# yigolden/JpegLibrary

Measured on AMD Instinct MI355X. Metric: Mpixels/s decoded, 4K 4:2:0 baseline Q75 RST=4, 1 & 8 GPU vs CPU ref, higher is better.
Workload: dtype f32; 1 GPU; 1024 x 3840x2160 420 baseline Q75 DRI=4 per GPU, output interleaved_u8 resident in HBM; images_per_gpu=1024

## Files before the change

jpeglibrary_amd/csrc/k3_idct.hip:

```cpp
#include <hip/hip_runtime.h>
#include <stdint.h>

#include <algorithm>
#include <atomic>
#include <cstdio>
#include <cstdlib>

#include "common.h"
#include "kernels.h"
#include "encode_kernels.h"
#include "kernels_device.h"

namespace jpgpu {


__device__ constexpr uint8_t kNat[64] = {0,  1,  8,  16, 9,  2,  3,  10, 17, 24, 32, 25, 18, 11, 4,  5,  12, 19, 26, 33, 40, 48,
                                         41, 34, 27, 20, 13, 6,  7,  14, 21, 28, 35, 42, 49, 56, 57, 50, 43, 36, 29, 22, 15, 23,
                                         30, 37, 44, 51, 58, 59, 52, 45, 38, 31, 39, 46, 53, 60, 61, 54, 47, 55, 62, 63};

static_assert(kIdctBlocksPerWg == 256, "the split form's reciprocals are exact for tiles of up to 256 blocks");
static_assert(kMaxBlocksPerMcu == 16, "kRecip16 and the 16-bit reciprocals of the split form cover 1..16 blocks per MCU");
__device__ constexpr uint32_t kRecip16[kMaxBlocksPerMcu + 1] = {0, 65536, 32768, 21846, 16384, 13108, 10923, 9363, 8192, 7282, 6554, 5958, 5462, 5042, 4682, 4370, 4096};

#define JPGPU_IDCT8(y0, y1, y2, y3, y4, y5, y6, y7)                     \
    {                                                                   \
        float mz0 = y1 + y7;                                            \
        float mz2 = y3 + y7;                                            \
        float mz1 = y3 + y5;                                            \
        float mz3 = y1 + y5;                                            \
        float mz4 = (mz0 + mz1) * 1.175875602f;                         \
        mz2 = (mz2 * -1.961570560f) + mz4;                              \
        mz3 = (mz3 * -0.390180644f) + mz4;                              \
        mz0 = mz0 * -0.899976223f;                                      \
        mz1 = mz1 * -2.562915447f;                                      \
        const float mb3 = ((y7 * 0.298631336f) + mz0) + mz2;            \
        const float mb2 = ((y5 * 2.053119869f) + mz1) + mz3;            \
        const float mb1 = ((y3 * 3.072711026f) + mz1) + mz2;            \
        const float mb0 = ((y1 * 1.501321110f) + mz0) + mz3;            \
        mz4 = (y2 + y6) * 0.541196100f;                                 \
        mz0 = y0 + y4;                                                  \
        mz1 = y0 - y4;                                                  \
        mz2 = mz4 + (y6 * -1.847759065f);                               \
        mz3 = mz4 + (y2 * 0.765366865f);                                \
        const float a0 = mz0 + mz3;                                     \
        const float a3 = mz0 - mz3;                                     \
        const float a1 = mz1 + mz2;                                     \
        const float a2 = mz1 - mz2;                                     \
        y0 = a0 + mb0;                                                  \
        y7 = a0 - mb0;                                                  \
        y1 = a1 + mb1;                                                  \
        y6 = a1 - mb1;                                                  \
        y2 = a2 + mb2;                                                  \
        y5 = a2 - mb2;                                                  \
        y3 = a3 + mb3;                                                  \
        y4 = a3 - mb3;                                                  \
    }

__device__ __forceinline__ void block_dequant(const uint8_t *c_lds, uint32_t swz, const uint16_t *q_lds, float (&f)[64]) {
#pragma unroll
    for (int piece = 0; piece < 8; piece++) {
        const uint4 cv = *reinterpret_cast<const uint4 *>(c_lds + ((piece ^ swz) * 16));
        const uint4 qv = reinterpret_cast<const uint4 *>(q_lds)[piece];
        const uint32_t cw[4] = {cv.x, cv.y, cv.z, cv.w};
        const uint32_t qw[4] = {qv.x, qv.y, qv.z, qv.w};
#pragma unroll
        for (int j = 0; j < 8; j++) {
            const int k = piece * 8 + j;
            const uint32_t w = cw[j >> 1], q = qw[j >> 1];
            const int32_t c = (j & 1) ? ((int32_t)w >> 16) : (int32_t)(int16_t)(w & 0xFFFF);
            const int32_t qq = (j & 1) ? (int32_t)(q >> 16) : (int32_t)(q & 0xFFFF);
            f[kNat[k]] = (float)(qq * c);
        }
    }
}

typedef float float2v __attribute__((ext_vector_type(2)));
typedef short short2v __attribute__((ext_vector_type(2)));
typedef unsigned short ushort2v __attribute__((ext_vector_type(2)));

template <typename T>
__device__ __forceinline__ void idct8(T &y0, T &y1, T &y2, T &y3, T &y4, T &y5, T &y6, T &y7) {
    T mz0 = y1 + y7;
    T mz2 = y3 + y7;
    T mz1 = y3 + y5;
    T mz3 = y1 + y5;
    T mz4 = (mz0 + mz1) * 1.175875602f;
    mz2 = (mz2 * -1.961570560f) + mz4;
    mz3 = (mz3 * -0.390180644f) + mz4;
    mz0 = mz0 * -0.899976223f;
    mz1 = mz1 * -2.562915447f;
    const T mb3 = ((y7 * 0.298631336f) + mz0) + mz2;
    const T mb2 = ((y5 * 2.053119869f) + mz1) + mz3;
    const T mb1 = ((y3 * 3.072711026f) + mz1) + mz2;
    const T mb0 = ((y1 * 1.501321110f) + mz0) + mz3;
// ... 127 lines not shown
            *reinterpret_cast<uint4 *>(dst + i * 4) = v;
        }
    } else {
        uint32_t w[N * 3 / 4];
#pragma unroll
        for (int i = 0; i < N; i += 4) {
            w[i * 3 / 4 + 0] = p[i] | (p[i + 1] << 24);
            w[i * 3 / 4 + 1] = (p[i + 1] >> 8) | (p[i + 2] << 16);
            w[i * 3 / 4 + 2] = (p[i + 2] >> 16) | (p[i + 3] << 8);
        }
        if (N == 16) {
#pragma unroll
            for (int i = 0; i < 3; i++) {
                const uint4 v = {w[i * 4], w[i * 4 + 1], w[i * 4 + 2], w[i * 4 + 3]};
                *reinterpret_cast<uint4 *>(dst + i * 16) = v;
            }
        } else {
#pragma unroll
            for (int i = 0; i < N * 3 / 8; i++) {
                const uint2 v = {w[i * 2], w[i * 2 + 1]};
                *reinterpret_cast<uint2 *>(dst + i * 8) = v;
            }
        }
    }
}

__global__ __launch_bounds__(256) void ycc_to_rgb_kernel(const uint8_t *__restrict__ src, uint8_t *__restrict__ dst, uint64_t n_pixels, int comps,
                                                         int bpp, YccRgbFactors k) {
    for (uint64_t i = (uint64_t)blockIdx.x * 256 + threadIdx.x; i < n_pixels; i += (uint64_t)gridDim.x * 256) {
        const uint32_t y = src[i * comps];
        const uint32_t cb = comps == 3 ? src[i * 3 + 1] : 128u, cr = comps == 3 ? src[i * 3 + 2] : 128u;
        const uint32_t px = rgb_pixel(y, chroma_terms(cb, cr, k));
        uint8_t *d = dst + i * bpp;
        d[0] = (uint8_t)px;
        d[1] = (uint8_t)(px >> 8);
        d[2] = (uint8_t)(px >> 16);
        if (bpp == 4) d[3] = 255;
    }
}

__global__ __launch_bounds__(256) void extend_u16_kernel(const uint8_t *__restrict__ planes, uint8_t *__restrict__ out_base,
                                                         const ExtendPlanes *__restrict__ images) {
    const ExtendPlanes g = images[blockIdx.y];
    uint16_t *out = reinterpret_cast<uint16_t *>(out_base + g.out_off);
    for (uint64_t px = (uint64_t)blockIdx.x * 256 + threadIdx.x; px < (uint64_t)g.width * g.height; px += (uint64_t)gridDim.x * 256) {
    const uint32_t y = (uint32_t)(px / g.width), x = (uint32_t)(px - (uint64_t)y * g.width);
    const uint32_t p = g.precision < 1u ? 1u : (g.precision > 16u ? 16u : g.precision), mx = (1u << p) - 1u;
    uint16_t v4[4] = {0, 0, 0, 0};
#pragma unroll
    for (uint32_t c = 0; c < 4u; c++) {
        if (c >= g.ncomp) continue;
        const int16_t *pl = reinterpret_cast<const int16_t *>(planes + g.plane_off[c]);
        const uint32_t mw = 8u * (g.max_h | (g.max_h == 0)), mh = 8u * (g.max_v | (g.max_v == 0));
        const uint32_t mcx = x / mw, pxm = x - mcx * mw, mcy = y / mh, pym = y - mcy * mh;
        const uint32_t bx = (pxm >> 3) < g.hcnt[c] - 1u ? (pxm >> 3) : g.hcnt[c] - 1u, by = (pym >> 3) < g.vcnt[c] - 1u ? (pym >> 3) : g.vcnt[c] - 1u;
        const uint32_t dx = pxm - 8u * bx, dy = pym - 8u * by;
        if (g.max_h != 0 && (dx >= (8u << g.hshift[c]) || dy >= (8u << g.vshift[c]))) continue;
        const uint32_t s = g.max_h == 0 ? (uint32_t)(uint16_t)pl[(uint64_t)(y >> g.vshift[c]) * g.pitch[c] + (x >> g.hshift[c])]
                                        : (uint32_t)(uint16_t)pl[(uint64_t)((mcy * g.vcnt[c] + by) * 8u + (dy >> g.vshift[c])) * g.pitch[c] + (mcx * g.hcnt[c] + bx) * 8u + (dx >> g.hshift[c])];
        uint32_t bits = s < mx ? s : mx;
        if (p >= 8u) {
            const uint32_t rem = 16u - p;
            bits = (bits << rem) | (bits & ((1u << rem) - 1u));
        } else {
            uint32_t cur = p;
            while (cur < 16u) {
                bits = (bits << p) | bits;
                cur += p;
            }
            if (cur > 16u) {
                bits >>= p;
                cur -= p;
                const uint32_t rem = 16u - cur;
                bits = (bits << rem) | (bits & ((1u << rem) - 1u));
            }
        }
        v4[c] = (uint16_t)bits;
    }
    *reinterpret_cast<uint2 *>(out + px * 4) = uint2{(uint32_t)v4[0] | ((uint32_t)v4[1] << 16), (uint32_t)v4[2] | ((uint32_t)v4[3] << 16)};
    }
}

template <int LAY, int CONV>
__device__ __forceinline__ void interleaved_output_from_tile(const uint8_t *sh_px, const DevScan &s, uint32_t tile_first, uint32_t n_mcu,
                                                             uint32_t tid, bool have_block, const DevScanComponent &comp, uint32_t mcu_x,
                                                             uint32_t mcu_y, uint32_t b, uint8_t *out, const YccRgbFactors &kf, bool reached,
                                                             uint32_t mcu, uint32_t fail_block) {
    const uint32_t W = s.width, H = s.height, C = s.frame_components;
    uint8_t *img = out + s.out_off;

    if (LAY == kLayGeneric) {
        if (have_block) {
            const uint32_t hs = comp.hs, vs = comp.vs;
            const bool flush = s.kind == kScanFrameOnly;
            const uint32_t x0 = flush ? (mcu_x * comp.h + s.blk_x[b]) * hs * 8 : (mcu_x * s.max_h + s.blk_x[b]) * 8;
            const uint32_t y0 = flush ? (mcu_y * comp.v + s.blk_y[b]) * vs * 8 : (mcu_y * s.max_v + s.blk_y[b]) * 8;
            const uint32_t hshift = 31 - __builtin_clz(hs | 1), vshift = 31 - __builtin_clz(vs | 1);
            const uint32_t bx = s.blk_x[b], by = s.blk_y[b];
            const bool overlap_h = !flush && comp.h > 1 && hs > 1, overlap_v = !flush && comp.v > 1 && vs > 1;
            const uint32_t base = b - (by * comp.h + bx);
            if ((overlap_h || overlap_v) && !reached) return;
            for (uint32_t v = 0; v < vs; v++)
                for (uint32_t i = 0; i < 8; i++) {
                    const uint32_t y = y0 + 8 * v + i;
                    if (y >= H) continue;
                    const uint8_t *srow = sh_px + ((8 * v + i) >> vshift) * kPxRowStride + tid * 8;
                    for (uint32_t h = 0; h < hs; h++) {
                        if (overlap_h || overlap_v) {
                            uint32_t later = 0xFFFFFFFFu;
                            if (overlap_h && bx + 1 < comp.h && h >= 1) later = base + by * comp.h + bx + 1;
                            else if (overlap_v && by + 1 < comp.v && v >= 1) {
                                const int32_t xf = (int32_t)bx + (int32_t)h - (int32_t)hs + 1;
                                later = base + (by + 1) * comp.h + (uint32_t)(xf < 0 ? 0 : xf);
                            }
                            if (later != 0xFFFFFFFFu && (uint64_t)mcu * s.blocks_per_mcu + later < fail_block) continue;
                        }
                        for (uint32_t j = 0; j < 8; j++) {
                            const uint32_t x = x0 + 8 * h + j;
                            if (x < W) img[((size_t)y * W + x) * C + comp.component_index] = srow[(8 * h + j) >> hshift];
                        }
                    }
                }
        }
    } else {
    constexpr uint32_t max_h = (LAY == kLayYccH1V1) ? 1 : 2;
    constexpr uint32_t max_v = (LAY == kLayYccH2V2) ? 2 : 1;
    constexpr uint32_t rows_per_mcu = 8 * max_v;
    constexpr uint32_t vshift = max_v >> 1;
    constexpr uint32_t kbpm = max_h * max_v + 2;
    const uint32_t n_tasks = rows_per_mcu * n_mcu;
    for (uint32_t t = tid; t < n_tasks; t += kIdctThreads) {
        const uint32_t row = t / n_mcu, m = t - row * n_mcu;
        const uint32_t gm = tile_first + m;
        const uint32_t gx = gm % s.mcus_per_line, gy = gm / s.mcus_per_line;
        const uint32_t y = gy * rows_per_mcu + row;
        if (y >= H) continue;
        const uint8_t *yrow = sh_px + (row & 7) * kPxRowStride + (m * kbpm + (row >> 3) * max_h) * 8;
        const uint8_t *crow = sh_px + (row >> vshift) * kPxRowStride + (m * kbpm + max_h * max_v) * 8;
        if (max_h == 2 && CONV != 0) {
            const uint4 yv = *reinterpret_cast<const uint4 *>(yrow);
            const uint4 cv = *reinterpret_cast<const uint4 *>(crow);
            uint32_t px[16];
#pragma unroll
            for (int j = 0; j < 8; j++) {
                const ChromaTerms t = chroma_terms(byte_of(cv.x, cv.y, j), byte_of(cv.z, cv.w, j), kf);
                px[2 * j] = rgb_pixel(byte_of(j < 4 ? yv.x : yv.z, j < 4 ? yv.y : yv.w, (2 * j) & 7), t);
                px[2 * j + 1] = rgb_pixel(byte_of(j < 4 ? yv.x : yv.z, j < 4 ? yv.y : yv.w, (2 * j + 1) & 7), t);
            }
            store_rgb_pixels<16, (CONV == 4 ? 4 : 3)>(img + ((size_t)y * W + gx * 16) * (CONV == 4 ? 4 : 3), px);
        } else if (CONV != 0) {
            const uint2 yv = *reinterpret_cast<const uint2 *>(yrow);
            const uint2 bv = *reinterpret_cast<const uint2 *>(crow);
            const uint2 rv = *reinterpret_cast<const uint2 *>(crow + 8);
            uint32_t px[8];
#pragma unroll
            for (int j = 0; j < 8; j++) px[j] = rgb_pixel(byte_of(yv.x, yv.y, j), chroma_terms(byte_of(bv.x, bv.y, j), byte_of(rv.x, rv.y, j), kf));
            store_rgb_pixels<8, (CONV == 4 ? 4 : 3)>(img + ((size_t)y * W + gx * 8) * (CONV == 4 ? 4 : 3), px);
        } else if (max_h == 2) {
            const uint4 yv = *reinterpret_cast<const uint4 *>(yrow);
            const uint4 cv = *reinterpret_cast<const uint4 *>(crow);
            const uint32_t cc0 = pick4(cv.x, cv.z, JPGPU_SEL(0, 4, 1, 5)), cc1 = pick4(cv.x, cv.z, JPGPU_SEL(2, 6, 3, 7));
            const uint32_t cc2 = pick4(cv.y, cv.w, JPGPU_SEL(0, 4, 1, 5)), cc3 = pick4(cv.y, cv.w, JPGPU_SEL(2, 6, 3, 7));
            uint4 o0, o1, o2;
            o0.x = pick4(yv.x, cc0, JPGPU_SEL(0, 4, 5, 1));
            o0.y = pick4(yv.x, cc0, JPGPU_SEL(4, 5, 2, 6));
            o0.z = pick4(yv.x, cc0, JPGPU_SEL(7, 3, 6, 7));
            o0.w = pick4(yv.y, cc1, JPGPU_SEL(0, 4, 5, 1));
            o1.x = pick4(yv.y, cc1, JPGPU_SEL(4, 5, 2, 6));
            o1.y = pick4(yv.y, cc1, JPGPU_SEL(7, 3, 6, 7));
            o1.z = pick4(yv.z, cc2, JPGPU_SEL(0, 4, 5, 1));
            o1.w = pick4(yv.z, cc2, JPGPU_SEL(4, 5, 2, 6));
            o2.x = pick4(yv.z, cc2, JPGPU_SEL(7, 3, 6, 7));
            o2.y = pick4(yv.w, cc3, JPGPU_SEL(0, 4, 5, 1));
            o2.z = pick4(yv.w, cc3, JPGPU_SEL(4, 5, 2, 6));
            o2.w = pick4(yv.w, cc3, JPGPU_SEL(7, 3, 6, 7));
            uint4 *dst = reinterpret_cast<uint4 *>(img + ((size_t)y * W + gx * 16) * 3);
            dst[0] = o0;
            dst[1] = o1;
            dst[2] = o2;
        } else {
            const uint2 yv = *reinterpret_cast<const uint2 *>(yrow);
            const uint2 bv = *reinterpret_cast<const uint2 *>(crow);
            const uint2 rv = *reinterpret_cast<const uint2 *>(crow + 8);
            uint2 o0, o1, o2;
            {
                const uint32_t lo = pick4(bv.x, rv.x, JPGPU_SEL(0, 4, 1, 5)), hi = pick4(bv.x, rv.x, JPGPU_SEL(2, 6, 3, 7));
                const uint32_t mid = pick4(lo, hi, JPGPU_SEL(2, 3, 4, 5));
                o0.x = pick4(yv.x, lo, JPGPU_SEL(0, 4, 5, 1));
                o0.y = pick4(yv.x, mid, JPGPU_SEL(4, 5, 2, 6));
                o1.x = pick4(yv.x, hi, JPGPU_SEL(5, 3, 6, 7));
            }
            {
                const uint32_t lo = pick4(bv.y, rv.y, JPGPU_SEL(0, 4, 1, 5)), hi = pick4(bv.y, rv.y, JPGPU_SEL(2, 6, 3, 7));
                const uint32_t mid = pick4(lo, hi, JPGPU_SEL(2, 3, 4, 5));
                o1.y = pick4(yv.y, lo, JPGPU_SEL(0, 4, 5, 1));
                o2.x = pick4(yv.y, mid, JPGPU_SEL(4, 5, 2, 6));
                o2.y = pick4(yv.y, hi, JPGPU_SEL(5, 3, 6, 7));
            }
            uint2 *dst = reinterpret_cast<uint2 *>(img + ((size_t)y * W + gx * 8) * 3);
            dst[0] = o0;
            dst[1] = o1;
            dst[2] = o2;
        }
    }
    }
}

typedef __attribute__((address_space(3))) void jpgpu_lds_void;
typedef const __attribute__((address_space(1))) void jpgpu_gbl_void;

template <int FMT, int LAY, bool PRE, bool SPLIT = false>
__device__ __forceinline__ void idct_output_body(
    const int16_t *__restrict__ coefs, const DevScan *__restrict__ scans, const IdctWork *__restrict__ work,
    const DevScanStatus *__restrict__ status, const DevQuantTable *__restrict__ quant_pool, uint8_t *__restrict__ out, YccRgbFactors kf) {
    constexpr int CONV = FMT == kFmtRgbU8 ? 3 : (FMT == kFmtRgbaU8 ? 4 : 0);
    constexpr bool kSampleBytes = fmt_is_sample_bytes(FMT);
    __shared__ __attribute__((aligned(16))) uint8_t sh_all[kIdctThreads * 128 + kIdctThreads * 64 + kMaxScanComponents * 128];
    uint8_t *sh = sh_all;
    uint8_t *sh_px = sh_all + kIdctThreads * 128;
    uint16_t(*sh_q)[64] = reinterpret_cast<uint16_t(*)[64]>(sh_all + kIdctThreads * 128 + kIdctThreads * 64);

    const IdctWork wk = work[blockIdx.x];
    const DevScan &s = scans[wk.scan];
    const uint32_t tid = threadIdx.x;
    const uint32_t wave = tid >> 6;
    const uint32_t bpm = s.blocks_per_mcu;
    const uint32_t mcus_per_tile = wk.mcus_per_tile;
    uint32_t decoded = status ? status[wk.scan].decoded_mcus : s.total_mcus;
    if (decoded > s.total_mcus) decoded = s.total_mcus;
    uint32_t fail_block = 0xFFFFFFFFu;
    if (status != nullptr && s.kind == kScanSequential) {
        const uint32_t fb = status[wk.scan].pad[1];
        if (fb != 0) fail_block = kFailBlockBase - fb;
        for (uint32_t j = s.first_scan; j < wk.scan; j++)
            if (scans[j].image_index == s.image_index && status[j].first_error != kNoError) fail_block = 0;
    }
    const bool keep = (s.shadow_mask & kKeepUnreachedMcus) != 0;
    constexpr bool kPerMcuLayout = fmt_is_interleaved(FMT) && (LAY == kLayYccH1V1 || LAY == kLayYccH2V1 || LAY == kLayYccH2V2);
    uint32_t first_mcu = wk.first_mcu;
    uint32_t range_end = wk.first_mcu + wk.n_mcus;
    if (first_mcu == kIdctPartialMcu) {
        if (fail_block == 0xFFFFFFFFu || fail_block % bpm == 0 || fail_block / bpm >= decoded) return;
        first_mcu = fail_block / bpm;
        range_end = first_mcu + 1;
    } else if (keep) {
        const uint32_t reach = kPerMcuLayout ? fail_block / bpm : (fail_block == 0xFFFFFFFFu ? fail_block : (fail_block + bpm - 1) / bpm);
        if (range_end > decoded) range_end = decoded;
        if (range_end > reach) range_end = reach;
        if (first_mcu >= range_end) return;
    }

    if (tid < (uint32_t)s.scan_components * 32) {
        const uint32_t c = tid >> 5, i = tid & 31;
        reinterpret_cast<uint32_t *>(sh_q[c])[i] =
            reinterpret_cast<const uint32_t *>(quant_pool[s.quant_pool[s.comp[c].quant_slot]].q)[i];
    }

    const uint32_t mcu_local = tid / bpm;
    const uint32_t b = tid - mcu_local * bpm;
    const uint32_t ci_early = s.blk_comp[b < kMaxBlocksPerMcu ? b : 0];
    const uint8_t *coef_bytes = reinterpret_cast<const uint8_t *>(coefs + s.coef_off * 64);

    auto tile_mcus = [&](uint32_t first) { return (range_end - first) < mcus_per_tile ? (range_end - first) : mcus_per_tile; };
    const uint32_t tile_blocks = mcus_per_tile * bpm;
    constexpr bool split = SPLIT && !PRE;
    if (split && (s.reserved0 & kScanSplitHandoff) == 0) return;
    const uint32_t sp_dri = split ? s.dri : 1u;
    const uint32_t sp_rb = kRecip16[bpm <= (uint32_t)kMaxBlocksPerMcu ? bpm : 0];
    const uint32_t sp_rd = __builtin_amdgcn_readfirstlane(sp_dri <= 256u ? ((1u << 20) + sp_dri - 1) / sp_dri : 0u);
    const uint32_t sp_w = sp_dri * bpm;
    const bool sp_fast = split && mcus_per_tile % (2 * sp_dri) == 0 && first_mcu % (2 * sp_dri) == 0;
    const uint32_t sp_rw = __builtin_amdgcn_readfirstlane((65536u + sp_w - 1) / sp_w);
    const uint8_t *sp_hi = coef_bytes + split_plane_lines(s.n_intervals, sp_dri, bpm) * 128;
    const uint8_t *sp_flags = reinterpret_cast<const uint8_t *>(reinterpret_cast<const uint64_t *>(coefs) + (s.reserved0 >> kSplitFlagShift));
    auto sp_locate = [&](uint32_t tile_first, uint32_t t, int k, uint32_t &line, uint32_t &iv, uint32_t &word) {
        const uint32_t i0 = __builtin_amdgcn_readfirstlane(tile_first / sp_dri), m0 = tile_first - i0 * sp_dri;
        const uint32_t blk = (uint32_t)k * 32 + (t >> 3);
        uint32_t q = (blk * sp_rb) >> 16;
        const uint32_t bb = blk - q * bpm;
        const uint32_t last = s.total_mcus - 1 - tile_first;
        q = q < last ? q : last;
        const uint32_t mm = m0 + q;
        const uint32_t by_mul = (mm * sp_rd) >> 20, by_cmp = mm >= sp_dri ? 1u : 0u;
        const uint32_t qi = sp_dri > 256u ? by_cmp : by_mul;
        const uint32_t m = mm - qi * sp_dri;
        iv = i0 + qi;
        line = ((iv >> 1) * sp_dri + m) * bpm + bb;
        word = ((iv >> 6) * sp_dri + m) * bpm + bb;
    };
    auto sp_locate_fast = [&](uint32_t i0, uint32_t t, int k, uint32_t &iv, uint32_t &word) {
        const uint32_t ll = (uint32_t)k * 16 + ((t >> 3) & 15u);
        const uint32_t pp = (ll * sp_rw) >> 16;
        iv = i0 + 2 * pp + ((t >> 7) & 1u);
        iv = iv < s.n_intervals ? iv : s.n_intervals - 1;
        word = (iv >> 6) * sp_w + (ll - pp * sp_w);
    };
    auto sp_own_block = [&](uint32_t t) {
        const uint32_t ml = (t * sp_rb) >> 16, bb = t - ml * bpm;
        const uint32_t ir = (ml * sp_rd) >> 20, m = ml - ir * sp_dri;
        const uint32_t ll = ((ir >> 1) * sp_dri + m) * bpm + bb;
        return ((ll >> 4) << 5) | ((ir & 1u) << 4) | (ll & 15u);
    };
    const uint32_t sp_ipt = __builtin_amdgcn_readfirstlane(mcus_per_tile / sp_dri);
    uint32_t sp_i0 = __builtin_amdgcn_readfirstlane(first_mcu / sp_dri);
    auto sp_load_flags = [&](uint32_t tile_first, uint32_t tile_i0, uint32_t (&fb)[8], uint32_t &bit_at) {
        uint32_t t_ = tid;
        asm volatile("" : "+v"(t_));
        bit_at = 0;
#pragma unroll
        for (int k = 0; k < 8; k++) {
            uint32_t line, iv, word;
            if (sp_fast) sp_locate_fast(tile_i0, t_, k, iv, word);
            else sp_locate(tile_first, t_, k, line, iv, word);
            fb[k] = sp_flags[word * 8 + ((iv >> 3) & 7u)];
            bit_at |= (iv & 7u) << (3 * k);
        }
    };
    auto sp_pack_flags = [&](uint32_t (&fb)[8], uint32_t bit_at) {
        uint32_t bits = 0;
#pragma unroll
        for (int k = 0; k < 8; k++) {
            asm volatile("" : "+v"(fb[k]));
            bits |= ((fb[k] >> ((bit_at >> (3 * k)) & 7u)) & 1u) << k;
        }
        return bits;
    };
    auto dma_tile = [&](uint32_t tile_first, uint32_t tile_i0, uint32_t hi_bits) {
        uint32_t t_ = tid;
        asm volatile("" : "+v"(t_));
        if (split && sp_fast) {
            const uint32_t piece = (t_ & 7) ^ ((t_ >> 4) & 7);
            const uint32_t slot = ((t_ >> 3) & 15u) * 2 + (t_ >> 7);
            const uint8_t *src = (piece < 4 ? coef_bytes : sp_hi) + (uint64_t)(tile_i0 >> 1) * sp_w * 128 + (slot * 64 + (piece & 3u) * 16);
            const uint8_t *zeros = sp_flags - 128 + (piece & 3u) * 16;
            const uint32_t fetch_bits = piece < 4 ? 0xFFu : hi_bits;
#pragma unroll
            for (int k = 0; k < 8; k++) {
                const uint8_t *from = ((fetch_bits >> k) & 1u) ? src + (uint32_t)(k * 2048) : zeros;
                if (k < 6 || (uint32_t)k * 32 + slot < tile_blocks)
                    __builtin_amdgcn_global_load_lds((jpgpu_gbl_void *)from, (jpgpu_lds_void *)(sh + ((uint32_t)k * kIdctThreads + wave * 64) * 16), 16, 0, 0);
            }
            return;
        }
        if (split) {
            const uint32_t piece = (t_ & 7) ^ ((t_ >> 4) & 7);
#pragma unroll
            for (int k = 0; k < 8; k++) {
                uint32_t line, iv, word;
                sp_locate(tile_first, t_, k, line, iv, word);
                const bool wanted = k < 6 || (uint32_t)k * 32 + (t_ >> 3) < tile_blocks;
                const bool fetch = wanted && (piece < 4 || ((hi_bits >> k) & 1u) != 0);
                const uint8_t *src = (piece < 4 ? coef_bytes : sp_hi) + ((uint64_t)line * 128 + (iv & 1u) * 64 + (piece & 3u) * 16);
                if (fetch)
                    __builtin_amdgcn_global_load_lds((jpgpu_gbl_void *)src, (jpgpu_lds_void *)(sh + ((uint32_t)k * kIdctThreads + wave * 64) * 16), 16, 0, 0);
                if (wanted && !fetch) *reinterpret_cast<uint4 *>(sh + ((uint32_t)k * kIdctThreads + t_) * 16) = uint4{0, 0, 0, 0};
            }
            return;
        }
        const uint32_t dma_lane_off = (t_ >> 3) * 128 + (((t_ & 7) ^ ((t_ >> 4) & 7)) * 16);
        const uint8_t *src = coef_bytes + (uint64_t)tile_first * bpm * 128;
#pragma unroll
        for (int k = 0; k < 8; k++)
            if (k < 6 || (uint32_t)k * 32 + (tid >> 3) < tile_blocks)
                __builtin_amdgcn_global_load_lds((jpgpu_gbl_void *)(src + (uint32_t)(k * 4096) + dma_lane_off),
                                                 (jpgpu_lds_void *)(sh + ((uint32_t)k * kIdctThreads + wave * 64) * 16), 16, 0, 0);
    };

    uint32_t hi_next = 0;
    if (split) {
        uint32_t fb[8], at;
        sp_load_flags(first_mcu, sp_i0, fb, at);
        asm volatile("s_waitcnt vmcnt(0)" ::: "memory");
        hi_next = sp_pack_flags(fb, at);
    }
    dma_tile(first_mcu, sp_i0, hi_next);
    if (split && first_mcu + mcus_per_tile < range_end) {
        uint32_t fb[8], at;
        sp_load_flags(first_mcu + mcus_per_tile, sp_i0 + sp_ipt, fb, at);
        asm volatile("s_waitcnt vmcnt(0)" ::: "memory");
        hi_next = sp_pack_flags(fb, at);
    }
    asm volatile("s_waitcnt vmcnt(0)" ::: "memory");
    __syncthreads();

  for (uint32_t tile_first = first_mcu; tile_first < range_end; tile_first += mcus_per_tile) {
    const uint32_t n_mcu = tile_mcus(tile_first);
    const uint32_t n_blk = n_mcu * bpm;
    const uint32_t next_first = tile_first + mcus_per_tile;
    const bool have_next = next_first < range_end;

    const uint32_t mcu = tile_first + mcu_local;
    const bool have_block = tid < n_blk;
    bool writes = have_block && ((s.shadow_mask >> ci_early) & 1u) == 0;

    float f[64];
    uint32_t px[32];
    if (PRE) {
        if (have_block) {
#pragma unroll
            for (int piece = 0; piece < 8; piece++) {
                const uint4 cv = *reinterpret_cast<const uint4 *>(sh + tid * 128 + ((piece ^ ((tid >> 1) & 7)) * 16));
                px[piece * 4] = cv.x;
                px[piece * 4 + 1] = cv.y;
                px[piece * 4 + 2] = cv.z;
                px[piece * 4 + 3] = cv.w;
            }
        }
    } else {
        constexpr bool kPerTile = split || (FMT == kFmtRgbU8 && (LAY == kLayYccH2V1 || LAY == kLayYccH2V2)) || (kSampleBytes && LAY == kLayGeneric);
        uint32_t t_ = tid;
        if (kPerTile) asm volatile("" : "+v"(t_));
        if (split && sp_fast) t_ = sp_own_block(t_);
        if (have_block) block_dequant(sh + t_ * 128, (t_ >> 1) & 7, sh_q[ci_early], f);
    }
    asm volatile("s_waitcnt lgkmcnt(0)" ::: "memory");
    __builtin_amdgcn_s_barrier();
    if (have_next) dma_tile(next_first, sp_i0 + sp_ipt, hi_next);
    hi_next = 0;

    if (!PRE && have_block) block_idct(f, (int32_t)s.level_shift, px);
    uint32_t sp_fb[8], sp_at = 0;
    const bool sp_ahead = split && next_first + mcus_per_tile < range_end;
    if (sp_ahead) sp_load_flags(next_first + mcus_per_tile, sp_i0 + 2 * sp_ipt, sp_fb, sp_at);
    sp_i0 += sp_ipt;
    const bool reached = mcu < decoded && mcu * bpm + b < fail_block;
    if ((s.shadow_mask & 0xFu) == 0) {
        writes = writes && (reached || !keep);
    } else {
        const uint32_t bb = b < kMaxBlocksPerMcu ? b : 0u, me = s.blk_comp[bb], fc = s.comp[me & 3u].component_index;
        uint32_t later = 0xFFu, earlier = 0xFFu;
        for (uint32_t cc = 0; cc < s.scan_components && cc < (uint32_t)kMaxScanComponents; cc++) {
            if (cc == me || s.comp[cc].component_index != fc) continue;
            if (cc > me && later == 0xFFu) later = cc;
            if (cc < me) earlier = cc;
        }
        uint32_t first_me = 0xFFu, first_later = 0xFFu, first_earlier = 0xFFu;
        for (uint32_t k = 0; k < bpm && k < (uint32_t)kMaxBlocksPerMcu; k++) {
            const uint32_t ck = s.blk_comp[k];
            if (ck == me && first_me == 0xFFu) first_me = k;
            if (ck == later && first_later == 0xFFu) first_later = k;
            if (ck == earlier && first_earlier == 0xFFu) first_earlier = k;
        }
        const bool later_reached = later != 0xFFu && mcu < decoded && mcu * bpm + (b - first_me + first_later) < fail_block;
        const bool earlier_reached = earlier != 0xFFu && mcu < decoded && mcu * bpm + (b - first_me + first_earlier) < fail_block;
        writes = have_block && (reached ? !later_reached : (!keep && later == 0xFFu && !earlier_reached));
    }
    if (!reached) {
#pragma unroll
        for (int i = 0; i < 32; i++) px[i] = 0;
    }
    bool synced = false;
    uint32_t mcu_late = mcu, b_late = b;
    asm volatile("" : "+v"(mcu_late), "+v"(b_late));
    const uint32_t mcu_y = mcu_late / s.mcus_per_line, mcu_x = mcu_late - mcu_y * s.mcus_per_line;
    const uint32_t ci = s.blk_comp[b_late < kMaxBlocksPerMcu ? b_late : 0];
    const DevScanComponent comp = s.comp[ci];
    const uint32_t b_out = split ? b_late : b;

    if (FMT == kFmtPlanarI16) {
        if (writes) {
            int16_t *plane = reinterpret_cast<int16_t *>(out + s.out_off + s.plane_off[ci]);
            const uint32_t pitch = s.plane_pitch[ci];
            const uint32_t x0 = (mcu_x * comp.h + s.blk_x[b_out]) * 8, y0 = (mcu_y * comp.v + s.blk_y[b_out]) * 8;
#pragma unroll
            for (int r = 0; r < 8; r++) {
                const uint4 v = {px[r * 4 + 0], px[r * 4 + 1], px[r * 4 + 2], px[r * 4 + 3]};
                *reinterpret_cast<uint4 *>(plane + (size_t)(y0 + r) * pitch + x0) = v;
            }
        }
    } else {
    uint2 rows[8];
    if constexpr (FMT == kFmtInterleavedU8Scaled) {
        const ScaleTo8 k8 = scale_to_8(s.precision);
        if (k8.expand) {
#pragma unroll
            for (int r = 0; r < 8; r++) {
                rows[r].x = __builtin_amdgcn_perm(expand2_u8(px[r * 4 + 1], k8), expand2_u8(px[r * 4 + 0], k8), 0x06040200u);
                rows[r].y = __builtin_amdgcn_perm(expand2_u8(px[r * 4 + 3], k8), expand2_u8(px[r * 4 + 2], k8), 0x06040200u);
            }
        } else {
#pragma unroll
            for (int r = 0; r < 8; r++) {
                rows[r].x = __builtin_amdgcn_perm(shift_sat2_u8(px[r * 4 + 1], k8), shift_sat2_u8(px[r * 4 + 0], k8), 0x05040100u);
                rows[r].y = __builtin_amdgcn_perm(shift_sat2_u8(px[r * 4 + 3], k8), shift_sat2_u8(px[r * 4 + 2], k8), 0x05040100u);
            }
        }
    } else {
#pragma unroll
    for (int r = 0; r < 8; r++) {
        rows[r].x = pack4_u8(px[r * 4 + 0], px[r * 4 + 1]);
        rows[r].y = pack4_u8(px[r * 4 + 2], px[r * 4 + 3]);
    }
    }

    if (CONV != 0 && LAY == kLayGray) {
        if (writes) {
            const uint32_t x0 = (mcu_x * comp.h + s.blk_x[b_out]) * 8, y0 = (mcu_y * comp.v + s.blk_y[b_out]) * 8;
#pragma unroll
            for (int r = 0; r < 8; r++) {
                if (y0 + r >= s.height) continue;
                uint32_t px[8];
#pragma unroll
                for (int j = 0; j < 8; j++) px[j] = byte_of(rows[r].x, rows[r].y, j) * 0x010101u;
                store_rgb_pixels<8, (CONV == 4 ? 4 : 3)>(out + s.out_off + ((size_t)(y0 + r) * s.width + x0) * (CONV == 4 ? 4 : 3), px);
            }
        }
    } else if (FMT == kFmtPlanarU8 || (kSampleBytes && LAY == kLayGray)) {
        if (writes) {
            const bool gray = kSampleBytes;
            uint8_t *plane = out + s.out_off + (gray ? 0 : s.plane_off[ci]);
            const uint32_t pitch = gray ? s.width : s.plane_pitch[ci];
            const uint32_t x0 = (mcu_x * comp.h + s.blk_x[b_out]) * 8, y0 = (mcu_y * comp.v + s.blk_y[b_out]) * 8;
#pragma unroll
            for (int r = 0; r < 8; r++)
                if (!gray || y0 + r < s.height) *reinterpret_cast<uint2 *>(plane + (size_t)(y0 + r) * pitch + x0) = rows[r];
        }
    } else {
    if (have_block) {
#pragma unroll
        for (int r = 0; r < 8; r++) *reinterpret_cast<uint2 *>(sh_px + r * kPxRowStride + tid * 8) = rows[r];
    }
    asm volatile("s_waitcnt vmcnt(0)\n\ts_waitcnt lgkmcnt(0)" ::: "memory");
    if (sp_ahead) hi_next = sp_pack_flags(sp_fb, sp_at);
    __builtin_amdgcn_s_barrier();
    synced = true;

    interleaved_output_from_tile<LAY, CONV>(sh_px, s, tile_first, n_mcu, tid, writes, comp, mcu_x, mcu_y, b, out, kf, reached, mcu, fail_block);
    }
    }

    if (!synced) {
        asm volatile("s_waitcnt vmcnt(0)\n\ts_waitcnt lgkmcnt(0)" ::: "memory");
        if (sp_ahead) hi_next = sp_pack_flags(sp_fb, sp_at);
        __builtin_amdgcn_s_barrier();
    }
  }
}


hipError_t launch_extend_u16(hipStream_t stream, const uint8_t *planes, uint8_t *out_base, const ExtendPlanes *images, int n_images,
                             uint32_t max_pixels) {
    if (n_images <= 0 || max_pixels == 0) return hipSuccess;
    const uint32_t bx = (uint32_t)std::min<uint64_t>(((uint64_t)max_pixels + 255) / 256, 4096);
    for (int base = 0; base < n_images; base += 65535) {
        const int n = n_images - base < 65535 ? n_images - base : 65535;
        hipLaunchKernelGGL(extend_u16_kernel, dim3(bx, (uint32_t)n), dim3(256), 0, stream, planes, out_base, images + base);
    }
    return hipGetLastError();
}


__global__ __launch_bounds__(256) void expand_handoff_kernel(const int16_t *__restrict__ coefs, int16_t *__restrict__ dense,
                                                             const DevScan *__restrict__ scans, const uint32_t *__restrict__ scan_ids) {
    const DevScan &s = scans[scan_ids[blockIdx.y]];
    const uint32_t bpm = s.blocks_per_mcu, dri = s.dri;
    const uint32_t n_blocks = s.total_mcus * bpm;
    const uint8_t *lo = reinterpret_cast<const uint8_t *>(coefs + s.coef_off * 64);
    const uint8_t *hi = lo + split_plane_lines(s.n_intervals, dri, bpm) * 128;
    const uint64_t *flags = reinterpret_cast<const uint64_t *>(coefs) + (s.reserved0 >> kSplitFlagShift);
    const uint32_t piece = threadIdx.x & 7;
    for (uint32_t g = blockIdx.x * 32 + (threadIdx.x >> 3); g < n_blocks; g += gridDim.x * 32) {
        const uint32_t mcu = g / bpm, b = g - mcu * bpm;
        const uint32_t i = mcu / dri, m = mcu - i * dri;
        const uint64_t off = split_slot(i, m, b, dri, bpm) * 64 + (piece & 3) * 16;
        uint4 v = {0, 0, 0, 0};
        if (piece < 4) v = *reinterpret_cast<const uint4 *>(lo + off);
        else if ((flags[split_flag_word(i, m, b, dri, bpm)] >> (i & 63u)) & 1u) v = *reinterpret_cast<const uint4 *>(hi + off);
        *reinterpret_cast<uint4 *>(dense + (s.coef_off + g) * 64 + piece * 8) = v;
    }
}
hipError_t launch_expand_handoff(hipStream_t stream, const int16_t *coefs, int16_t *dense, const DevScan *scans, const uint32_t *scan_ids, int n_scans,
                                 uint32_t max_blocks) {
    if (n_scans <= 0 || max_blocks == 0) return hipSuccess;
    const uint32_t bx = (uint32_t)std::min<uint64_t>(((uint64_t)max_blocks + 31) / 32, 2048);
    for (int base = 0; base < n_scans; base += 65535) {
        const int n = n_scans - base < 65535 ? n_scans - base : 65535;
        hipLaunchKernelGGL(expand_handoff_kernel, dim3(bx, (uint32_t)n), dim3(256), 0, stream, coefs, dense, scans, scan_ids + base);
    }
    return hipGetLastError();
}

template <int FMT, int LAY>
__global__ __launch_bounds__(kIdctThreads, (FMT == kFmtPlanarI16 ? 2 : 3)) void idct_output_kernel(
    const int16_t *__restrict__ coefs, const DevScan *__restrict__ scans, const IdctWork *__restrict__ work,
    const DevScanStatus *__restrict__ status, const DevQuantTable *__restrict__ quant_pool, uint8_t *__restrict__ out, YccRgbFactors kf) {
    idct_output_body<FMT, LAY, false>(coefs, scans, work, status, quant_pool, out, kf);
}
template <int FMT, int LAY>
__global__ __launch_bounds__(kIdctThreads, (FMT == kFmtPlanarI16 ? 2 : 3)) void idct_split_kernel(
    const int16_t *__restrict__ coefs, const DevScan *__restrict__ scans, const IdctWork *__restrict__ work,
    const DevScanStatus *__restrict__ status, const DevQuantTable *__restrict__ quant_pool, uint8_t *__restrict__ out, YccRgbFactors kf) {
    idct_output_body<FMT, LAY, false, true>(coefs, scans, work, status, quant_pool, out, kf);
}
template <int FMT>
__global__ __launch_bounds__(kIdctThreads, 2) void flush_output_kernel(
    const int16_t *__restrict__ coefs, const DevScan *__restrict__ scans, const IdctWork *__restrict__ work,
    const DevScanStatus *__restrict__ status, const DevQuantTable *__restrict__ quant_pool, uint8_t *__restrict__ out, YccRgbFactors kf) {
    idct_output_body<FMT, kLayGeneric, true>(coefs, scans, work, status, quant_pool, out, kf);
}

__global__ __launch_bounds__(64) void dispose_pass_kernel(int16_t *__restrict__ coefs, const DisposeJob *__restrict__ jobs,
                                                          const DevQuantTable *__restrict__ quant_pool) {
    const DisposeJob &j = jobs[blockIdx.y];
    const uint32_t g = blockIdx.x * 64u + threadIdx.x;
    if (g >= j.n_blocks) return;
    const uint32_t c = j.blk_comp[g % j.bpm];
    const uint32_t n = j.n[c];
    if (n == 0) return;
    int16_t *blk = coefs + (j.coef_off + g) * 64;
    uint32_t w[32];
#pragma unroll
    for (int i = 0; i < 8; i++) {
        const uint4 v = reinterpret_cast<const uint4 *>(blk)[i];
        w[i * 4] = v.x;
        w[i * 4 + 1] = v.y;
        w[i * 4 + 2] = v.z;
        w[i * 4 + 3] = v.w;
    }
// ... 118 lines not shown
```

Baseline: 605,400 Mpixels/s.

## Replace per-task integer division with reciprocal index math and ballot-shared split flags

```diff
diff --git a/jpeglibrary_amd/csrc/k3_idct.hip b/jpeglibrary_amd/csrc/k3_idct.hip
--- a/jpeglibrary_amd/csrc/k3_idct.hip
+++ b/jpeglibrary_amd/csrc/k3_idct.hip
@@ -10,6 +10,7 @@
 #include "kernels.h"
 #include "encode_kernels.h"
 #include "kernels_device.h"
+#include "k3_index_math.h"
 
 namespace jpgpu {
 
@@ -303,14 +304,13 @@
 }
 
 template <int LAY, int CONV>
-__device__ __forceinline__ void interleaved_output_from_tile(const uint8_t *sh_px, const DevScan &s, uint32_t tile_first, uint32_t n_mcu,
+__device__ __forceinline__ void interleaved_output_from_tile(const uint8_t *sh_px, const DevScan &s, const K3TilePos &pos, uint32_t mpl,
+                                                             uint32_t line_recip, uint32_t row_recip, uint32_t img_h, uint32_t n_mcu,
                                                              uint32_t tid, bool have_block, const DevScanComponent &comp, uint32_t mcu_x,
-                                                             uint32_t mcu_y, uint32_t b, uint8_t *out, const YccRgbFactors &kf, bool reached,
+                                                             uint32_t mcu_y, uint32_t b, uint8_t *img, const YccRgbFactors &kf, bool reached,
                                                              uint32_t mcu, uint32_t fail_block) {
-    const uint32_t W = s.width, H = s.height, C = s.frame_components;
-    uint8_t *img = out + s.out_off;
-
     if (LAY == kLayGeneric) {
+        const uint32_t W = s.width, H = s.height, C = s.frame_components;
         if (have_block) {
             const uint32_t hs = comp.hs, vs = comp.vs;
             const bool flush = s.kind == kScanFrameOnly;
@@ -349,15 +349,23 @@
     constexpr uint32_t rows_per_mcu = 8 * max_v;
     constexpr uint32_t vshift = max_v >> 1;
     constexpr uint32_t kbpm = max_h * max_v + 2;
+    constexpr uint32_t bpp = CONV == 4 ? 4 : 3;
     const uint32_t n_tasks = rows_per_mcu * n_mcu;
+    const uint32_t W = mpl * (8 * max_h);
+    const uint32_t y0 = pos.gy0 * rows_per_mcu;
+    uint8_t *line0 = img + (uint64_t)y0 * W * bpp;
     for (uint32_t t = tid; t < n_tasks; t += kIdctThreads) {
-        const uint32_t row = t / n_mcu, m = t - row * n_mcu;
-        const uint32_t gm = tile_first + m;
-        const uint32_t gx = gm % s.mcus_per_line, gy = gm / s.mcus_per_line;
-        const uint32_t y = gy * rows_per_mcu + row;
-        if (y >= H) continue;
-        const uint8_t *yrow = sh_px + (row & 7) * kPxRowStride + (m * kbpm + (row >> 3) * max_h) * 8;
-        const uint8_t *crow = sh_px + (row >> vshift) * kPxRowStride + (m * kbpm + max_h * max_v) * 8;
+        const uint32_t row = k3_task_row(t, row_recip), m = t - k3_mul24(row, n_mcu);
+        const uint32_t x = pos.gx0 + m, wraps = k3_line_wraps(x, mpl, line_recip);
+        uint32_t back = k3_mul24(wraps, mpl);
+        asm("" : "+v"(back));
+        const uint32_t gx = x - back;
+        const uint32_t yl = wraps * rows_per_mcu + row;
+        if (y0 + yl >= img_h) continue;
+        const uint32_t mb = k3_mul24(m, kbpm);
+        const uint8_t *yrow = sh_px + (row & 7) * kPxRowStride + (mb + (row >> 3) * max_h) * 8;
+        const uint8_t *crow = sh_px + (row >> vshift) * kPxRowStride + (mb + max_h * max_v) * 8;
+        uint8_t *dst_px = line0 + (k3_mul24(yl, W * bpp) + k3_mul24(gx, 8 * max_h * bpp));
         if (max_h == 2 && CONV != 0) {
             const uint4 yv = *reinterpret_cast<const uint4 *>(yrow);
             const uint4 cv = *reinterpret_cast<const uint4 *>(crow);
@@ -368,7 +376,7 @@
                 px[2 * j] = rgb_pixel(byte_of(j < 4 ? yv.x : yv.z, j < 4 ? yv.y : yv.w, (2 * j) & 7), t);
                 px[2 * j + 1] = rgb_pixel(byte_of(j < 4 ? yv.x : yv.z, j < 4 ? yv.y : yv.w, (2 * j + 1) & 7), t);
             }
-            store_rgb_pixels<16, (CONV == 4 ? 4 : 3)>(img + ((size_t)y * W + gx * 16) * (CONV == 4 ? 4 : 3), px);
+            store_rgb_pixels<16, bpp>(dst_px, px);
         } else if (CONV != 0) {
             const uint2 yv = *reinterpret_cast<const uint2 *>(yrow);
             const uint2 bv = *reinterpret_cast<const uint2 *>(crow);
@@ -376,7 +384,7 @@
             uint32_t px[8];
 #pragma unroll
             for (int j = 0; j < 8; j++) px[j] = rgb_pixel(byte_of(yv.x, yv.y, j), chroma_terms(byte_of(bv.x, bv.y, j), byte_of(rv.x, rv.y, j), kf));
-            store_rgb_pixels<8, (CONV == 4 ? 4 : 3)>(img + ((size_t)y * W + gx * 8) * (CONV == 4 ? 4 : 3), px);
+            store_rgb_pixels<8, bpp>(dst_px, px);
         } else if (max_h == 2) {
             const uint4 yv = *reinterpret_cast<const uint4 *>(yrow);
             const uint4 cv = *reinterpret_cast<const uint4 *>(crow);
@@ -395,7 +403,7 @@
             o2.y = pick4(yv.w, cc3, JPGPU_SEL(0, 4, 5, 1));
             o2.z = pick4(yv.w, cc3, JPGPU_SEL(4, 5, 2, 6));
             o2.w = pick4(yv.w, cc3, JPGPU_SEL(7, 3, 6, 7));
-            uint4 *dst = reinterpret_cast<uint4 *>(img + ((size_t)y * W + gx * 16) * 3);
+            uint4 *dst = reinterpret_cast<uint4 *>(dst_px);
             dst[0] = o0;
             dst[1] = o1;
             dst[2] = o2;
@@ -418,7 +426,7 @@
                 o2.x = pick4(yv.y, mid, JPGPU_SEL(4, 5, 2, 6));
                 o2.y = pick4(yv.y, hi, JPGPU_SEL(5, 3, 6, 7));
             }
-            uint2 *dst = reinterpret_cast<uint2 *>(img + ((size_t)y * W + gx * 8) * 3);
+            uint2 *dst = reinterpret_cast<uint2 *>(dst_px);
             dst[0] = o0;
             dst[1] = o1;
             dst[2] = o2;
@@ -436,10 +444,11 @@
     const DevScanStatus *__restrict__ status, const DevQuantTable *__restrict__ quant_pool, uint8_t *__restrict__ out, YccRgbFactors kf) {
     constexpr int CONV = FMT == kFmtRgbU8 ? 3 : (FMT == kFmtRgbaU8 ? 4 : 0);
     constexpr bool kSampleBytes = fmt_is_sample_bytes(FMT);
-    __shared__ __attribute__((aligned(16))) uint8_t sh_all[kIdctThreads * 128 + kIdctThreads * 64 + kMaxScanComponents * 128];
+    __shared__ __attribute__((aligned(16))) uint8_t sh_all[kIdctThreads * 128 + kIdctThreads * 64 + kMaxScanComponents * 128 + (SPLIT && !PRE ? 64 : 0)];
     uint8_t *sh = sh_all;
     uint8_t *sh_px = sh_all + kIdctThreads * 128;
     uint16_t(*sh_q)[64] = reinterpret_cast<uint16_t(*)[64]>(sh_all + kIdctThreads * 128 + kIdctThreads * 64);
+    uint8_t *sh_flag = sh_all + kIdctThreads * 128 + kIdctThreads * 64 + kMaxScanComponents * 128;
 
     const IdctWork wk = work[blockIdx.x];
     const DevScan &s = scans[wk.scan];
@@ -494,9 +503,9 @@
     const uint32_t sp_rw = __builtin_amdgcn_readfirstlane((65536u + sp_w - 1) / sp_w);
     const uint8_t *sp_hi = coef_bytes + split_plane_lines(s.n_intervals, sp_dri, bpm) * 128;
     const uint8_t *sp_flags = reinterpret_cast<const uint8_t *>(reinterpret_cast<const uint64_t *>(coefs) + (s.reserved0 >> kSplitFlagShift));
-    auto sp_locate = [&](uint32_t tile_first, uint32_t t, int k, uint32_t &line, uint32_t &iv, uint32_t &word) {
+    auto sp_locate = [&](uint32_t tile_first, uint32_t t, uint32_t k, uint32_t &line, uint32_t &iv, uint32_t &word) {
         const uint32_t i0 = __builtin_amdgcn_readfirstlane(tile_first / sp_dri), m0 = tile_first - i0 * sp_dri;
-        const uint32_t blk = (uint32_t)k * 32 + (t >> 3);
+        const uint32_t blk = k * 32 + (t >> 3);
         uint32_t q = (blk * sp_rb) >> 16;
         const uint32_t bb = blk - q * bpm;
         const uint32_t last = s.total_mcus - 1 - tile_first;
@@ -509,8 +518,8 @@
         line = ((iv >> 1) * sp_dri + m) * bpm + bb;
         word = ((iv >> 6) * sp_dri + m) * bpm + bb;
     };
-    auto sp_locate_fast = [&](uint32_t i0, uint32_t t, int k, uint32_t &iv, uint32_t &word) {
-        const uint32_t ll = (uint32_t)k * 16 + ((t >> 3) & 15u);
+    auto sp_locate_fast = [&](uint32_t i0, uint32_t t, uint32_t k, uint32_t &iv, uint32_t &word) {
+        const uint32_t ll = k * 16 + ((t >> 3) & 15u);
         const uint32_t pp = (ll * sp_rw) >> 16;
         iv = i0 + 2 * pp + ((t >> 7) & 1u);
         iv = iv < s.n_intervals ? iv : s.n_intervals - 1;
@@ -524,26 +533,31 @@
     };
     const uint32_t sp_ipt = __builtin_amdgcn_readfirstlane(mcus_per_tile / sp_dri);
     uint32_t sp_i0 = __builtin_amdgcn_readfirstlane(first_mcu / sp_dri);
-    auto sp_load_flags = [&](uint32_t tile_first, uint32_t tile_i0, uint32_t (&fb)[8], uint32_t &bit_at) {
+    auto sp_load_flag = [&](uint32_t tile_first, uint32_t tile_i0, uint32_t &fb, uint32_t &bit_at) {
         uint32_t t_ = tid;
         asm volatile("" : "+v"(t_));
-        bit_at = 0;
-#pragma unroll
-        for (int k = 0; k < 8; k++) {
-            uint32_t line, iv, word;
-            if (sp_fast) sp_locate_fast(tile_i0, t_, k, iv, word);
-            else sp_locate(tile_first, t_, k, line, iv, word);
-            fb[k] = sp_flags[word * 8 + ((iv >> 3) & 7u)];
-            bit_at |= (iv & 7u) << (3 * k);
-        }
+        const uint32_t k = t_ >> 5, t8 = (t_ & 31u) << 3;
+        uint32_t line, iv, word;
+        if (sp_fast) sp_locate_fast(tile_i0, t8, k, iv, word);
+        else sp_locate(tile_first, t8, k, line, iv, word);
+        fb = sp_flags[word * 8 + ((iv >> 3) & 7u)];
+        bit_at = iv & 7u;
     };
-    auto sp_pack_flags = [&](uint32_t (&fb)[8], uint32_t bit_at) {
+    auto sp_wait_seen = [&]() {
+        if (split) __builtin_amdgcn_s_waitcnt(0x0070);
+    };
+    auto sp_publish_flags = [&](uint32_t fb, uint32_t bit_at, uint32_t set) {
+        asm volatile("" : "+v"(fb));
+        const uint64_t w = __builtin_amdgcn_ballot_w64(((fb >> bit_at) & 1u) != 0);
+        if ((tid & 63u) == 0) *reinterpret_cast<uint2 *>(sh_flag + set * 32 + wave * 8) = uint2{(uint32_t)w, (uint32_t)(w >> 32)};
+    };
+    auto sp_read_flags = [&](uint32_t set) {
+        const uint4 lo = *reinterpret_cast<const uint4 *>(sh_flag + set * 32), hi = *reinterpret_cast<const uint4 *>(sh_flag + set * 32 + 16);
+        const uint32_t w[8] = {lo.x, lo.y, lo.z, lo.w, hi.x, hi.y, hi.z, hi.w};
+        const uint32_t at = tid >> 3;
         uint32_t bits = 0;
 #pragma unroll
-        for (int k = 0; k < 8; k++) {
-            asm volatile("" : "+v"(fb[k]));
-            bits |= ((fb[k] >> ((bit_at >> (3 * k)) & 7u)) & 1u) << k;
-        }
+        for (int k = 0; k < 8; k++) bits |= ((w[k] >> at) & 1u) << k;
         return bits;
     };
     auto dma_tile = [&](uint32_t tile_first, uint32_t tile_i0, uint32_t hi_bits) {
@@ -589,18 +603,34 @@
 
     uint32_t hi_next = 0;
     if (split) {
-        uint32_t fb[8], at;
-        sp_load_flags(first_mcu, sp_i0, fb, at);
-        asm volatile("s_waitcnt vmcnt(0)" ::: "memory");
-        hi_next = sp_pack_flags(fb, at);
-    }
-    dma_tile(first_mcu, sp_i0, hi_next);
-    if (split && first_mcu + mcus_per_tile < range_end) {
-        uint32_t fb[8], at;
-        sp_load_flags(first_mcu + mcus_per_tile, sp_i0 + sp_ipt, fb, at);
-        asm volatile("s_waitcnt vmcnt(0)" ::: "memory");
-        hi_next = sp_pack_flags(fb, at);
-    }
+        const uint32_t n_sets = first_mcu + mcus_per_tile < range_end ? 2u : 1u;
+#pragma nounroll
+        for (uint32_t set = 0; set < n_sets; set++) {
+            uint32_t fb, at;
+            sp_load_flag(first_mcu + set * mcus_per_tile, sp_i0 + set * sp_ipt, fb, at);
+            asm volatile("s_waitcnt vmcnt(0)" ::: "memory");
+            sp_wait_seen();
+            sp_publish_flags(fb, at, set);
+        }
+        __syncthreads();
+        const uint32_t hi_first = sp_read_flags(0);
+        if (n_sets == 2) hi_next = sp_read_flags(1);
+        dma_tile(first_mcu, sp_i0, hi_first);
+    } else {
+        dma_tile(first_mcu, sp_i0, 0);
+    }
+    const uint32_t mpl = __builtin_amdgcn_readfirstlane(s.mcus_per_line);
+    const uint32_t line_recip = __builtin_amdgcn_readfirstlane(k3_line_recip(mpl));
+    const uint32_t img_h = __builtin_amdgcn_readfirstlane((uint32_t)s.height);
+    uint8_t *const img = out + s.out_off;
+    K3TilePos pos = k3_tile_pos(first_mcu, mpl);
+    pos.gx0 = __builtin_amdgcn_readfirstlane(pos.gx0);
+    pos.gy0 = __builtin_amdgcn_readfirstlane(pos.gy0);
+    K3TilePos pos_step = k3_tile_pos(mcus_per_tile, mpl);
+    pos_step.gx0 = __builtin_amdgcn_readfirstlane(pos_step.gx0);
+    pos_step.gy0 = __builtin_amdgcn_readfirstlane(pos_step.gy0);
+    const uint32_t row_recip_full = __builtin_amdgcn_readfirstlane(k3_row_recip(mcus_per_tile));
+    const uint32_t row_recip_last = __builtin_amdgcn_readfirstlane(k3_row_recip((range_end - first_mcu - 1) % mcus_per_tile + 1));
     asm volatile("s_waitcnt vmcnt(0)" ::: "memory");
     __syncthreads();
 
@@ -640,9 +670,9 @@
     hi_next = 0;
 
     if (!PRE && have_block) block_idct(f, (int32_t)s.level_shift, px);
-    uint32_t sp_fb[8], sp_at = 0;
+    uint32_t sp_fb = 0, sp_at = 0;
     const bool sp_ahead = split && next_first + mcus_per_tile < range_end;
-    if (sp_ahead) sp_load_flags(next_first + mcus_per_tile, sp_i0 + 2 * sp_ipt, sp_fb, sp_at);
+    if (sp_ahead) sp_load_flag(next_first + mcus_per_tile, sp_i0 + 2 * sp_ipt, sp_fb, sp_at);
     sp_i0 += sp_ipt;
     const bool reached = mcu < decoded && mcu * bpm + b < fail_block;
     if ((s.shadow_mask & 0xFu) == 0) {
@@ -671,9 +701,12 @@
         for (int i = 0; i < 32; i++) px[i] = 0;
     }
     bool synced = false;
-    uint32_t mcu_late = mcu, b_late = b;
-    asm volatile("" : "+v"(mcu_late), "+v"(b_late));
-    const uint32_t mcu_y = mcu_late / s.mcus_per_line, mcu_x = mcu_late - mcu_y * s.mcus_per_line;
+    uint32_t ml_late = mcu_local, b_late = b;
+    asm volatile("" : "+v"(ml_late), "+v"(b_late));
+    const uint32_t mcu_wraps = k3_line_wraps(pos.gx0 + ml_late, mpl, line_recip);
+    uint32_t mcu_back = k3_mul24(mcu_wraps, mpl);
+    asm("" : "+v"(mcu_back));
+    const uint32_t mcu_y = pos.gy0 + mcu_wraps, mcu_x = pos.gx0 + ml_late - mcu_back;
     const uint32_t ci = s.blk_comp[b_late < kMaxBlocksPerMcu ? b_late : 0];
     const DevScanComponent comp = s.comp[ci];
     const uint32_t b_out = split ? b_late : b;
@@ -742,19 +775,26 @@
         for (int r = 0; r < 8; r++) *reinterpret_cast<uint2 *>(sh_px + r * kPxRowStride + tid * 8) = rows[r];
     }
     asm volatile("s_waitcnt vmcnt(0)\n\ts_waitcnt lgkmcnt(0)" ::: "memory");
-    if (sp_ahead) hi_next = sp_pack_flags(sp_fb, sp_at);
+    sp_wait_seen();
+    if (sp_ahead) sp_publish_flags(sp_fb, sp_at, 0);
+    asm volatile("s_waitcnt lgkmcnt(0)" ::: "memory");
     __builtin_amdgcn_s_barrier();
     synced = true;
 
-    interleaved_output_from_tile<LAY, CONV>(sh_px, s, tile_first, n_mcu, tid, writes, comp, mcu_x, mcu_y, b, out, kf, reached, mcu, fail_block);
+    interleaved_output_from_tile<LAY, CONV>(sh_px, s, pos, mpl, line_recip, n_mcu == mcus_per_tile ? row_recip_full : row_recip_last, img_h, n_mcu, tid,
+                                            writes, comp, mcu_x, mcu_y, b, img, kf, reached, mcu, fail_block);
     }
     }
 
     if (!synced) {
         asm volatile("s_waitcnt vmcnt(0)\n\ts_waitcnt lgkmcnt(0)" ::: "memory");
-        if (sp_ahead) hi_next = sp_pack_flags(sp_fb, sp_at);
+        sp_wait_seen();
+        if (sp_ahead) sp_publish_flags(sp_fb, sp_at, 0);
+        asm volatile("s_waitcnt lgkmcnt(0)" ::: "memory");
         __builtin_amdgcn_s_barrier();
     }
+    if (sp_ahead) hi_next = sp_read_flags(0);
+    k3_tile_advance(pos, pos_step, mpl);
   }
 }
 
diff --git a/jpeglibrary_amd/csrc/k3_index_math.h b/jpeglibrary_amd/csrc/k3_index_math.h
--- /dev/null
+++ b/jpeglibrary_amd/csrc/k3_index_math.h
@@ -0,0 +1,53 @@
+#pragma once
+#include <stdint.h>
+
+#ifndef JPGPU_HD
+#if defined(__HIPCC__) || defined(__CUDACC__)
+#define JPGPU_HD __host__ __device__
+#else
+#define JPGPU_HD
+#endif
+#endif
+
+namespace jpgpu {
+
+constexpr uint32_t kK3MaxTileMcus = 85;
+constexpr uint32_t kK3MaxTileLanes = 256;
+constexpr uint32_t kK3LineRecipBelow = 256;
+
+JPGPU_HD inline uint32_t k3_mul24(uint32_t a, uint32_t b) {
+#if defined(__HIP_DEVICE_COMPILE__)
+    return __umul24(a, b);
+#else
+    return (a & 0xFFFFFFu) * (b & 0xFFFFFFu);
+#endif
+}
+
+JPGPU_HD inline uint32_t k3_row_recip(uint32_t n_mcu) { return ((1u << 20) + n_mcu - 1u) / (n_mcu | (n_mcu == 0)); }
+JPGPU_HD inline uint32_t k3_task_row(uint32_t t, uint32_t row_recip) { return k3_mul24(t, row_recip) >> 20; }
+
+JPGPU_HD inline uint32_t k3_line_recip(uint32_t mcus_per_line) {
+    return mcus_per_line < kK3LineRecipBelow ? ((1u << 20) + mcus_per_line - 1u) / (mcus_per_line | (mcus_per_line == 0)) : 0u;
+}
+JPGPU_HD inline uint32_t k3_line_wraps(uint32_t x, uint32_t mcus_per_line, uint32_t line_recip) {
+    const uint32_t by_mul = k3_mul24(x, line_recip) >> 20, by_cmp = x >= mcus_per_line ? 1u : 0u;
+    return mcus_per_line < kK3LineRecipBelow ? by_mul : by_cmp;
+}
+
+struct K3TilePos {
+    uint32_t gx0, gy0;
+};
+JPGPU_HD inline K3TilePos k3_tile_pos(uint32_t first_mcu, uint32_t mcus_per_line) {
+    const uint32_t gy0 = first_mcu / mcus_per_line;
+    return K3TilePos{first_mcu - gy0 * mcus_per_line, gy0};
+}
+JPGPU_HD inline void k3_tile_advance(K3TilePos &p, const K3TilePos &step, uint32_t mcus_per_line) {
+    p.gx0 += step.gx0;
+    p.gy0 += step.gy0;
+    if (p.gx0 >= mcus_per_line) {
+        p.gx0 -= mcus_per_line;
+        p.gy0 += 1;
+    }
+}
+
+}
```

Measured after the change: 633,500 Mpixels/s (median of 6 runs). 4.6% higher.
